# dan11003/tbv_slam_public

Hardware: AMD Instinct MI355X
Metric: radar scan registrations/sec (400x3360 polar) (higher is better)
Workload: dtype u8 filter / f32 search / f64 solve

## Files before the change

include/cfear_hip.h:

```cpp
#ifndef CFEAR_HIP_H
#define CFEAR_HIP_H
#include <stddef.h>
#include <stdint.h>

#ifdef __cplusplus
extern "C" {
#endif

#define CFEAR_ABI_VERSION 1

#define CFEAR_OK 0
#define CFEAR_ERR_INVALID_ARGUMENT (-1)
#define CFEAR_ERR_HIP (-2)
#define CFEAR_ERR_CAPACITY (-3)
#define CFEAR_ERR_TOO_FEW_RESIDUALS (-4)
#define CFEAR_ERR_SOLVER (-5)
#define CFEAR_ERR_EMPTY_CLOUD (-6)
#define CFEAR_ERR_NO_DEVICE (-7)
#define CFEAR_ERR_IO (-8)
#define CFEAR_ERR_FORMAT (-9)

enum cfear_cost_metric { CFEAR_P2P = 0, CFEAR_P2L = 1, CFEAR_P2D = 2 };
enum cfear_loss_type { CFEAR_LOSS_NONE = 0, CFEAR_LOSS_HUBER = 1, CFEAR_LOSS_CAUCHY = 2,
                       CFEAR_LOSS_SOFTLONE = 3, CFEAR_LOSS_COMBINED = 4,
// ... 204 lines not shown
#define CFEAR_SURF_REASON_ROTATION 2u
#define CFEAR_SURF_REASON_POINTS 3u
#define CFEAR_SURF_REASON_CELLS 4u
#define CFEAR_SURF_REASON_ORDER 5u
#define CFEAR_SURF_REASON_ROWS3 6u
#define CFEAR_SURF_PATH_SLAB_COUNT_SHIFT 16
#define CFEAR_SURF_PATH_SLAB_COUNT_MASK 0xFF0000u
int cfear_scan_destroy(cfear_scan* scan);

typedef struct cfear_scan_batch cfear_scan_batch;
int cfear_scan_create_batch(cfear_ctx* ctx, const float* xyzi, const int64_t* offsets, const int32_t* lengths, int32_t n_scans,
                            const cfear_feature_params* par, const double* mots, int32_t max_cells, cfear_scan_batch** out,
                            int32_t* status);
int cfear_scan_batch_size(const cfear_scan_batch* batch);
int cfear_scan_batch_get(const cfear_scan_batch* batch, int32_t i, const cfear_scan** scan);
int cfear_scan_batch_destroy(cfear_scan_batch* batch);

typedef struct cfear_reg_params {
  int32_t cost;
  int32_t loss;
  double loss_limit;
  int32_t weight_opt;
  int32_t max_itr_association;
  int32_t max_itr_solver;
  int32_t min_itr;
  double radius;
  double cov_scale;
  double regularization;
  double score_tolerance;
  int32_t itr;
// ... 717 lines not shown
```

tbv_slam_public_amd/_lib.py:

```python
import ctypes as C
import os

import numpy as np

_HERE = os.path.dirname(os.path.abspath(__file__))
SO_PATH = os.path.join(_HERE, "libcfear_hip.so")

OK = 0
ERR_INVALID_ARGUMENT, ERR_HIP, ERR_CAPACITY = -1, -2, -3
ERR_TOO_FEW_RESIDUALS, ERR_SOLVER, ERR_EMPTY_CLOUD, ERR_NO_DEVICE = -4, -5, -6, -7
ERR_IO, ERR_FORMAT = -8, -9

P2P, P2L, P2D = 0, 1, 2
LOSS = {"None": 0, "Huber": 1, "Cauchy": 2, "SoftLOne": 3, "Combined": 4, "Tukey": 5}
COST = {"P2P": 0, "P2L": 1, "P2D": 2}

SURF_PATH_KIND_MASK, SURF_PATH_FAST, SURF_PATH_SINGLE, SURF_PATH_GLOBAL = 3, 1, 2, 3
SURF_PATH_ROWS, SURF_PATH_K64, SURF_PATH_WFLOAT, SURF_PATH_SLABS, SURF_PATH_READ2 = 0x4, 0x8, 0x10, 0x20, 0x40
SURF_PATH_TIER16, SURF_PATH_TIER4, SURF_PATH_TIER1, SURF_PATH_TOP_BUCKET, SURF_PATH_CEN_SCRATCH = 0x80, 0x100, 0x200, 0x400, 0x800
SURF_PATH_PREPARED, SURF_PATH_REASON_SHIFT, SURF_PATH_REASON_MASK = 0x1000, 13, 0xE000
SURF_REASON_REACH, SURF_REASON_ROTATION, SURF_REASON_POINTS, SURF_REASON_CELLS, SURF_REASON_ORDER, SURF_REASON_ROWS3 = 1, 2, 3, 4, 5, 6
SURF_PATH_SLAB_COUNT_SHIFT, SURF_PATH_SLAB_COUNT_MASK = 16, 0xFF0000


# ... 296 lines not shown
    "cfear_rccl_unique_id", "cfear_rccl_comm_init", "cfear_rccl_comm_destroy",
    "cfear_candidate_pipe_create", "cfear_candidate_pipe_submit", "cfear_candidate_pipe_collect", "cfear_candidate_pipe_destroy", "cfear_candidate_pipe_stats",
    "cfear_eval_params_default", "cfear_eval_trajectories", "cfear_eval_check", "cfear_kitti_read", "cfear_kitti_write",
    "cfear_kitti_from_xyt", "cfear_cen2018_params_default", "cfear_filter_cen2018",
    "cfear_cen2019_params_default", "cfear_filter_cen2019",
    "cfear_logreg_params_default", "cfear_logreg_fit_batch", "cfear_p2p_quality", "cfear_p2p_quality_batch",
    "cfear_cart_params_default", "cfear_polar_to_cartesian", "cfear_cart_quality_batch",
    "cfear_cacfar_plan", "cfear_filter_cacfar_rowkeys", "cfear_kstrong_plan",
    "cfear_closure_params_default", "cfear_closure_candidates_batch",
    "cfear_loop_stats_params_default", "cfear_loop_stats_batch", "cfear_loop_curves_params_default", "cfear_loop_curves_batch",
    "cfear_sync_trajectories", "cfear_tum_write", "cfear_cov_write",
    "cfear_graph_align_batch", "cfear_graph_map_batch", "cfear_graph_string_write", "cfear_graph_output_write",
    "cfear_association_ties_batch", "cfear_scan_closest_ties",
    "cfear_voxel_audit_params_default", "cfear_voxel_order_audit_batch",
    "cfear_cen2019_order_audit",
    "cfear_scan_create_batch", "cfear_scan_batch_size", "cfear_scan_batch_get", "cfear_scan_batch_destroy",
    "cfear_odometry_replay_clouds", "cfear_odometry_replay",
    "cfear_sc_detect_batch",
    "cfear_kstrong_rowkeys_derive",
    "cfear_odometry_grid_plan", "cfear_odometry_grid_create", "cfear_odometry_grid_process", "cfear_odometry_grid_destroy",
]


class RowkeysClass(C.Structure):
    _fields_ = [("image", C.c_int32), ("k_strongest", C.c_int32), ("z_min", C.c_float), ("range_res", C.c_float),
                ("min_distance", C.c_float)]


GRID_STREAM_DTYPE = np.dtype([(n, "<i4") for n in ("sequence", "config", "sweep", "filter_class", "surface_group", "matcher_group",
                                                   "surface_slot", "matcher_slot")])

# ... 254 lines not shown
    L.cfear_sc_detect_sequence.argtypes = [vp, C.POINTER(ScManagerParams), C.POINTER(ScNode), C.c_int32, C.c_int32, C.c_int32,
                                           vp, vp]
    L.cfear_sc_detect_batch.argtypes = [vp, C.POINTER(ScManagerParams), C.POINTER(ScBatch), vp, vp]
    L.cfear_sc_manager_size.argtypes = [vp]
    L.cfear_sc_manager_destroy.argtypes = [vp]
    L.cfear_scan_closest_idx.argtypes = [vp, vp, C.c_int32, C.c_double, vp]
    L.cfear_scan_closest_ties.argtypes = [vp, vp, C.c_int32, C.c_double, vp, vp, vp]
    L.cfear_association_ties_batch.argtypes = [vp, C.POINTER(RegJob), C.c_int32, C.POINTER(RegParams), C.c_int32, vp, vp, C.c_int64]
    L.cfear_voxel_audit_params_default.argtypes = [C.POINTER(VoxelAuditParams)]
    L.cfear_voxel_audit_params_default.restype = None
    L.cfear_voxel_order_audit_batch.argtypes = [vp, vp, vp, vp, C.c_int32, C.POINTER(VoxelAuditParams), vp, vp, C.c_int64, C.POINTER(C.c_int64)]
    L.cfear_scan_surface_path.argtypes = [vp, C.POINTER(C.c_uint32)]
    L.cfear_scan_create_batch.argtypes = [vp, vp, vp, vp, C.c_int32, C.POINTER(FeatureParams), vp, C.c_int32, C.POINTER(vp), vp]
    L.cfear_scan_batch_size.argtypes = [vp]
    L.cfear_scan_batch_get.argtypes = [vp, C.c_int32, C.POINTER(vp)]
    L.cfear_scan_batch_destroy.argtypes = [vp]
    L.cfear_odometry_replay_clouds.argtypes = [vp, C.POINTER(ScCloud), C.POINTER(OdometryParams), vp, vp, C.c_int32, C.c_int32, vp]
    L.cfear_odometry_replay.argtypes = [vp, C.POINTER(PolarDesc), vp, C.POINTER(OdometryParams), vp, vp, C.c_int32, C.c_int32, vp]
    L.cfear_polar_rotate_ccw.argtypes = [vp, vp, C.POINTER(PolarDesc), vp, C.c_int32, C.c_int64]
    L.cfear_verify_params_default.argtypes = [C.POINTER(VerifyParams)]
    L.cfear_verify_params_default.restype = None
    L.cfear_verify_loop_candidates.argtypes = [vp, C.POINTER(VerifyJob), C.c_int32, C.POINTER(VerifyParams), vp]
    L.cfear_verify_apply_constraints.argtypes = [vp, C.c_int32, C.POINTER(VerifyParams), vp]
    L.cfear_verify_by_odometry.argtypes = [vp, C.c_int32, C.c_double, C.c_int32, C.POINTER(C.c_double)]
    L.cfear_get_cost.argtypes = [vp, C.POINTER(vp), C.c_int32, C.POINTER(C.c_double), C.POINTER(RegParams),
                                 C.POINTER(C.c_double), C.POINTER(C.c_double), C.c_int32,
                                 C.POINTER(C.c_int32), C.POINTER(C.c_double)]
    L.cfear_cost_prepare.argtypes = [vp, C.POINTER(vp), C.c_int32, C.POINTER(C.c_double),
                                     C.POINTER(RegParams), C.c_int32, C.POINTER(vp)]
    L.cfear_cost_num_blocks.argtypes = [vp]
# ... 94 lines not shown
```

tbv_slam_public_amd/api.py:

```python
import ctypes as C
import math
import os

import numpy as np

from . import _lib as L


def _is_torch(x):
    return type(x).__module__.startswith("torch")


def _ptr(x):
    if x is None:
        return None, None
    if _is_torch(x):
        assert x.is_contiguous()
        return x.data_ptr(), x
    assert x.flags["C_CONTIGUOUS"]
    return x.ctypes.data, x


def _torch_ready(ctx, *arrays):
    if not any(_is_torch(a) for a in arrays):
# ... 527 lines not shown
            ctx.check(ctx._lib.cfear_scan_batch_get(h, i, C.byref(s)))
            m = None
            if s.value:
                m = MapPointNormal._from_handle(s, ctx)
                m._batch = self
            self._scans.append(m)

    def __len__(self):
        return len(self._scans)

    def __getitem__(self, i):
        return self._scans[i]

    def __iter__(self):
        return iter(self._scans)

    def close(self):
        if getattr(self, "_h", None):
            for m in self._scans:
                if m is not None:
                    m._h, m._batch = None, None
            if getattr(self.ctx, "h", None):
                self.ctx._lib.cfear_scan_batch_destroy(self._h)
            self._h = None

    def __del__(self):
        try:
            self.close()
        except Exception:
            pass
# ... 3149 lines not shown
```

tbv_slam_public_amd/csrc/common.hpp:

```cpp
#pragma once
#include <hip/hip_runtime.h>

#include <cstddef>
#include <cstdint>
#include <cstdio>
#include <cstring>
#include <initializer_list>
#include <map>
#include <string>
#include <type_traits>
#include <vector>

#include "../../include/cfear_hip.h"
#include "batch_tables.hpp"
#include "owned.hpp"
#include "reg_layout.hpp"

#define CFEAR_WAVE 64

template <class T> using DevBuf = Owned<T, hipFree>;
template <class T> using PinnedBuf = Owned<T[], hipHostFree>;
using Event = Owned<std::remove_pointer_t<hipEvent_t>, hipEventDestroy>;
using Stream = Owned<std::remove_pointer_t<hipStream_t>, hipStreamDestroy>;
using GraphExec = Owned<std::remove_pointer_t<hipGraphExec_t>, hipGraphExecDestroy>;
// ... 237 lines not shown
  DevBuf<void> slab;
  ScanView view;
  int32_t n_cells_host;
  uint32_t surf_path = 0;
  int32_t refs = 1;
  cfear_scan_batch* batch = nullptr;
};
void cfear_scan_retain(cfear_scan* scan);
int cfear_scan_release(cfear_scan* scan);

struct cfear_scan_batch {
  cfear_ctx* ctx = nullptr;
  DevBuf<void> arena;
  size_t arena_bytes = 0;
  std::vector<cfear_scan*> scans;
  int32_t live = 0;
  bool released = false;
};
void cfear_scan_batch_free(cfear_scan_batch* b);
int cfear_scan_batch_build(cfear_ctx* ctx, const float* const* clouds, const char* on_host, bool one_buffer, const int32_t* lengths, int n_scans,
                           const cfear_feature_params* par, const double* mots, int max_cells, cfear_scan_batch** out, int32_t* status);

size_t cfear_scan_slab_bytes(int cap);
ScanView cfear_scan_view(void* slab, int cap);
int cfear_scan_alloc(cfear_ctx* ctx, int cap, cfear_scan** out);
int cfear_scan_clone_view(cfear_ctx* ctx, const ScanView& src, int n_cells, cfear_scan** out);

struct cfear_kstrong_fused {
  uint32_t* row_keys = nullptr;
  int32_t* row_valid = nullptr;
// ... 166 lines not shown
```

tbv_slam_public_amd/csrc/surface.hip:

```cpp
#include <cfloat>
#include <cmath>
#include <memory>
#include <type_traits>

#include "common.hpp"
#include "fastmath.hpp"
#include "gridsort.hpp"

namespace {

constexpr int kSurfThreads = kGridSortThreads;
constexpr int kMaxPoints = kGridSortMaxPoints;
constexpr int kMaxGridRows = 4096;
constexpr int kPerThread = kMaxPoints / kSurfThreads;
constexpr size_t kLdsRowbegOff = (size_t)kMaxPoints * 8 + 16;
constexpr size_t kLdsSmallOff = (kLdsRowbegOff + (size_t)(kMaxGridRows + 1) * 4 + 15) / 16 * 16;
constexpr size_t kLdsTotal = kLdsSmallOff + 256 + 64 + 32;

struct SurfJob {
  float4* xyzi;
  const int32_t* n_ptr;
  int32_t n_host;
  int32_t compensate;
  double mot[3];
// ... 218 lines not shown
  if (!cov_reasonable) return 0;
  double n0 = vmin[0], n1 = vmin[1];
  if (n0 * (ox - u0) + n1 * (oy - u1) < 0) { n0 = -n0; n1 = -n1; }
  tc.mean[0] = u0; tc.mean[1] = u1;
  tc.normal[0] = n0; tc.normal[1] = n1;
  tc.cov[0] = c00; tc.cov[1] = c01; tc.cov[2] = c10; tc.cov[3] = c11;
  tc.scale = log(1.0 + condition_number / 2);
  tc.avg_intensity = sum_intensity / (double)m.cnt;
  tc.lmin = lmin; tc.lmax = lmax;
  tc.nsamples = m.cnt;
  tc.valid = 1;
  return 1;
}

constexpr size_t kScanGridLds = (size_t)kScanGridCells * 4 + 128;
__device__ void grid_cells_block(const ScanView& v, int n, uint8_t* lds) {
  const int tid = threadIdx.x, nth = blockDim.x;
  unsigned* cnt = (unsigned*)lds;
  unsigned* ext = cnt + kScanGridCells;
  auto ordered = [](float f) { unsigned u = __float_as_uint(f); return (u >> 31) ? ~u : (u | 0x80000000u); };
  auto unordered = [](unsigned u) { return __uint_as_float((u >> 31) ? (u & 0x7fffffffu) : ~u); };
  if (n > 65535) {
    if (tid == 0) *v.grid_geo = make_float4(0.f, 0.f, 0.f, 0.f);
    return;
  }
  const int np = scan_grid_pad(n);
  unsigned short* cstart = v.grid;
  float2* rec_xy = (float2*)(v.grid + kScanGridStartPad);
  unsigned short* rec_idx = (unsigned short*)(rec_xy + np);
  for (int c = tid; c < kScanGridCells; c += nth) cnt[c] = 0;
  if (tid < 4) ext[tid] = (tid & 1) ? 0u : 0xFFFFFFFFu;
  __syncthreads();
  {
    unsigned xl = 0xFFFFFFFFu, xh = 0u, yl = 0xFFFFFFFFu, yh = 0u;
    for (int i = tid; i < n; i += nth) {
      const g_f32x2 m = gload<g_f32x2>(v.mean_f + i);
      const unsigned ux = ordered(m.x), uy = ordered(m.y);
      xl = min(xl, ux); xh = max(xh, ux); yl = min(yl, uy); yh = max(yh, uy);
    }
    for (int o = 32; o > 0; o >>= 1) {
      xl = min(xl, (unsigned)__shfl_xor((int)xl, o)); xh = max(xh, (unsigned)__shfl_xor((int)xh, o));
      yl = min(yl, (unsigned)__shfl_xor((int)yl, o)); yh = max(yh, (unsigned)__shfl_xor((int)yh, o));
    }
    if ((tid & 63) == 0) { atomicMin(&ext[0], xl); atomicMax(&ext[1], xh); atomicMin(&ext[2], yl); atomicMax(&ext[3], yh); }
  }
  __syncthreads();
  float x0 = 0.f, y0 = 0.f, span = 0.f;
  if (n > 0) {
    x0 = unordered(ext[0]); y0 = unordered(ext[2]);
    span = fmaxf(unordered(ext[1]) - x0, unordered(ext[3]) - y0);
  }
  const float inv = 1.0f / fmaxf(span / (float)kScanGrid * 1.0001f, kScanGridMinEdge);
  auto cell_of = [&](float x, float y) {
    const int cx = min(kScanGrid - 1, max(0, (int)floorf((x - x0) * inv)));
    const int cy = min(kScanGrid - 1, max(0, (int)floorf((y - y0) * inv)));
    return cy * kScanGrid + cx;
  };
  for (int i = tid; i < n; i += nth) { const g_f32x2 m = gload<g_f32x2>(v.mean_f + i); atomicAdd(&cnt[cell_of(m.x, m.y)], 1u); }
  __syncthreads();
  {
    const int per = (kScanGridCells + nth - 1) / nth, c0 = tid * per, c1 = min(kScanGridCells, c0 + per);
    int tot = 0;
    for (int c = c0; c < c1; c++) tot += (int)cnt[c];
    const int incl = wave_incl_scan_i32(tot);
    if ((tid & 63) == 63) ext[4 + (tid >> 6)] = (unsigned)incl;
    __syncthreads();
    int run = incl - tot;
    for (int wv = 0; wv < (tid >> 6); wv++) run += (int)ext[4 + wv];
    for (int c = c0; c < c1; c++) {
      const int k = (int)cnt[c];
      gstore<unsigned short>(cstart + c, (unsigned short)run);
      cnt[c] = (unsigned)run;
      run += k;
    }
    if (tid < kScanGridStartPad - kScanGridCells) gstore<unsigned short>(cstart + kScanGridCells + tid, (unsigned short)n);
  }
  __syncthreads();
  for (int i = tid; i < n; i += nth) {
    const g_f32x2 m = gload<g_f32x2>(v.mean_f + i);
    const unsigned pos = atomicAdd(&cnt[cell_of(m.x, m.y)], 1u);
    gstore<g_f32x2>(rec_xy + pos, m);
    gstore<unsigned short>(rec_idx + pos, (unsigned short)i);
  }
  if (tid < np - n) {
    gstore<g_f32x2>(rec_xy + n + tid, g_f32x2{0.f, 0.f});
    gstore<unsigned short>(rec_idx + n + tid, (unsigned short)0);
  }
  if (tid == 0) gstore<g_f32x4>(v.grid_geo, g_f32x4{x0, y0, inv, 1.f});
}

__global__ __launch_bounds__(kSurfThreads) void scan_grid_kernel(ScanView v) {
  __shared__ __attribute__((aligned(16))) uint8_t smem[kScanGridLds];
  grid_cells_block(v, *v.n_cells, smem);
}

__device__ void surface_big_tail(const SurfJob& job, const SurfCommon& cm, const int job_id, const int n, const int dbx,
                                 const int dby, const int min_bx, const int min_by, uint8_t* smem) {
  int* red_i = (int*)(smem + kLdsSmallOff + 256);
  const int tid = threadIdx.x, wave = tid >> 6, lane = tid & 63;
  const SurfScratch scr = scratch_of(cm.scratch + (size_t)job_id * cm.scratch_stride, cm.scratch_cap);
  const float4* pts = job.xyzi;
  unsigned long long* keys = scr.bigkeys;
  int npad = 1024;
  while (npad < n) npad <<= 1;
  for (int i = tid; i < npad; i += kSurfThreads) {
    unsigned long long key = ~0ull;
    if (i < n) {
      const float4 p = pts[i];
// ... 348 lines not shown
        job.out.mean[off] = make_double2(t.mean[0], t.mean[1]);
        job.out.normal[off] = make_double2(t.normal[0], t.normal[1]);
        job.out.cov[off] = make_double4(t.cov[0], t.cov[1], t.cov[2], t.cov[3]);
        job.out.scale[off] = t.scale;
        job.out.avg_intensity[off] = t.avg_intensity;
        job.out.lambda[off] = make_double2(t.lmin, t.lmax);
        job.out.nsamples[off] = t.nsamples;
      }
    }
    __syncthreads();
    if (tid == 0) { int tot = 0; for (int wv = 0; wv < 16; wv++) tot += red_i[wv]; sh_misc[0] += tot; }
    __syncthreads();
  }
  __threadfence_block();
  __syncthreads();
  grid_cells_block(job.out, min(sh_misc[0], job.out.cap), smem);
  if (tid == 0) {
    const int total = sh_misc[0];
    *job.out.n_cells = total <= job.out.cap ? total : job.out.cap;
    *status = total <= job.out.cap ? CFEAR_OK : CFEAR_ERR_CAPACITY;
    if (cm.ncells_out) cm.ncells_out[job_id] = total <= job.out.cap ? total : job.out.cap;
    if (cm.path_out) cm.path_out[job_id] = path;
  }
}

__global__ __launch_bounds__(kSurfThreads) void surface_points_kernel(const SurfJob* __restrict__ jobs, const SurfCommon cm) {
  extern __shared__ __attribute__((aligned(16))) uint8_t smem[];
  if (!cm.fallback) { surface_points_job(jobs, cm, blockIdx.x, smem); return; }
  const int count = min(cm.fallback[0], cm.n_jobs);
  for (int w = blockIdx.x; w < count; w += gridDim.x) {
    surface_points_job(jobs, cm, cm.fallback[1 + w], smem);
// ... 574 lines not shown
    scr.hdr->n = n; scr.hdr->V = V; scr.hdr->dbx = dbx; scr.hdr->dby = dby;
    scr.hdr->path = path | (n_slabs > 1 ? CFEAR_SURF_PATH_SLABS : 0u) | ((uint32_t)min(n_slabs, 255) << CFEAR_SURF_PATH_SLAB_COUNT_SHIFT);
  }
}

__global__ __launch_bounds__(kFastThreads, 4) void surface_sort_kernel(const SurfJob* __restrict__ jobs, const SurfCommon cm) {
  surface_sort_job<32>(jobs, cm);
}
__global__ __launch_bounds__(kFastThreads, 4) void surface_sort_mixed_kernel(const SurfJob* __restrict__ jobs, const SurfCommon cm) {
  const SurfScratch scr = scratch_of(cm.scratch + (size_t)blockIdx.x * cm.scratch_stride, cm.scratch_cap);
  if (scr.hdr->n > 32 * kFastThreads) surface_sort_job<64>(jobs, cm);
  else surface_sort_job<32>(jobs, cm);
}

constexpr int kFinishThreads = 256;

__global__ __launch_bounds__(kFinishThreads, 5) void surface_finish_kernel(const SurfJob* __restrict__ jobs, const SurfCommon cm) {
  extern __shared__ __attribute__((aligned(16))) uint8_t smem[];
  __shared__ int red_i2[2][kFinishThreads / 64];
  const int tid = threadIdx.x, wave = tid >> 6, lane = tid & 63;
  const int job_id = blockIdx.x;
  const SurfScratch scr = scratch_of(cm.scratch + (size_t)job_id * cm.scratch_stride, cm.scratch_cap);
  if (job_id == 0 && tid == 0) cm.fallback[0] = 0;
  if (scr.hdr->route != kRouteFast) return;
  const SurfJob job = jobs[job_id];
  const int V = scr.hdr->V;
  int run = 0;
  int cnt_next = tid < V ? gload<int32_t>(scr.coff + tid) : 0;
  for (int v0 = 0, rnd = 0; v0 < V; v0 += kFinishThreads, rnd ^= 1) {
    const int v = v0 + tid;
    const int cnt = cnt_next;
    cnt_next = v + kFinishThreads < V ? gload<int32_t>(scr.coff + v + kFinishThreads) : 0;
    TmpCell t;
    int f = 0;
    if (v < V && cnt >= 6) {
      const char* src = (const char*)&scr.tmp[v];
      const g_f64x2 a = gload<g_f64x2>(src), b = gload<g_f64x2>(src + 16), c = gload<g_f64x2>(src + 32);
      const g_f32x2 d = gload<g_f32x2>(src + 48);
      const Moments mo{cnt, a.x, a.y, b.x, b.y, c.x, c.y};
      f = finish_cell(mo, (double)d.x, (double)d.y, cm.origin[0], cm.origin[1], t);
    }
    const int inc = wave_incl_scan_i32(f);
    if (lane == 63) red_i2[rnd][wave] = inc;
    __syncthreads();
    int off = run + inc - f;
    for (int wv = 0; wv < kFinishThreads / 64; wv++) { if (wv < wave) off += red_i2[rnd][wv]; run += red_i2[rnd][wv]; }
    if (f && off < job.out.cap) {
      gstore<g_f32x2>(job.out.mean_f + off, g_f32x2{(float)t.mean[0], (float)t.mean[1]});
      gstore<g_f64x2>(job.out.mean + off, g_f64x2{t.mean[0], t.mean[1]});
      gstore<g_f64x2>(job.out.normal + off, g_f64x2{t.normal[0], t.normal[1]});
      gstore<g_f64x4>(job.out.cov + off, g_f64x4{t.cov[0], t.cov[1], t.cov[2], t.cov[3]});
      gstore<double>(job.out.scale + off, t.scale);
      gstore<double>(job.out.avg_intensity + off, t.avg_intensity);
      gstore<g_f64x2>(job.out.lambda + off, g_f64x2{t.lmin, t.lmax});
      gstore<int32_t>(job.out.nsamples + off, t.nsamples);
    }
  }
  __threadfence_block();
  __syncthreads();
  const int total = run;
  const int cap = min(job.out.cap, cm.finish_keys);
  grid_cells_block(job.out, min(total, cap), smem);
  if (tid == 0) {
    *job.out.n_cells = total <= cap ? total : cap;
    cm.status[job_id] = total <= cap ? CFEAR_OK : CFEAR_ERR_CAPACITY;
    if (cm.ncells_out) cm.ncells_out[job_id] = total <= cap ? total : cap;
    if (cm.path_out) cm.path_out[job_id] = scr.hdr->path;
  }
}

__global__ void cells_to_slab_kernel(const cfear_cell* cells, int n, ScanView v) {
  const int i = blockIdx.x * blockDim.x + threadIdx.x;
  if (i == 0) *v.n_cells = n;
  if (i >= n) return;
  const cfear_cell c = cells[i];
  v.mean_f[i] = make_float2((float)c.mean[0], (float)c.mean[1]);
  v.mean[i] = make_double2(c.mean[0], c.mean[1]);
  v.normal[i] = make_double2(c.normal[0], c.normal[1]);
  v.cov[i] = make_double4(c.cov[0], c.cov[1], c.cov[2], c.cov[3]);
  v.scale[i] = c.scale;
  v.avg_intensity[i] = c.avg_intensity;
  v.lambda[i] = make_double2(c.lambda_min, c.lambda_max);
  v.nsamples[i] = c.nsamples;
}
// ... 71 lines not shown
  cm.range_res = polar ? polar->range_res : 0.0;
  cm.range_off = polar ? polar->range_off : 0.0;
  cm.n_jobs = n_jobs;
  cm.fast_ok = cm.reach == 1 ? 1 : 0;
  const size_t ws_bytes_before = ctx->ws[kWsSurfaceList].bytes;
  cm.fallback = (int32_t*)cfear_workspace(ctx, kWsSurfaceList, ((size_t)n_jobs + 16) * 4);
  if (!cm.fallback) return cfear_set_error(ctx, CFEAR_ERR_HIP, "workspace allocation failed");
  if (ctx->ws[kWsSurfaceList].bytes != ws_bytes_before || ctx->surf_list_dirty)
    CFEAR_HIP_CHECK(ctx, hipMemsetAsync(cm.fallback, 0, 4, ctx->stream));
  ctx->surf_list_dirty = true;
  { const int rc_lds = cfear_allow_lds(ctx, (const void*)surface_points_kernel, cfear_surface_lds_bytes()); if (rc_lds != CFEAR_OK) return rc_lds; }
  { const int rc_lds = cfear_allow_lds(ctx, (const void*)surface_sort_kernel, kFastLds); if (rc_lds != CFEAR_OK) return rc_lds; }
  const bool big_scans = cap_points > kMaxPoints;
  if (big_scans) { const int rc_lds = cfear_allow_lds(ctx, (const void*)surface_sort_mixed_kernel, kFastLds); if (rc_lds != CFEAR_OK) return rc_lds; }
  cm.finish_keys = std::min(max_cell_cap, kMaxPoints);
  const size_t finish_lds = kScanGridLds;
  cm.finish_lds = (uint32_t)finish_lds;
  {
    size_t prep_lds = 0;
    if (polar) {
      const size_t np = (size_t)std::min<long long>((long long)polar->rows * polar->k, kFastMaxPoints);
      prep_lds = (((size_t)(polar->rows + 1) * 4 + 15) & ~(size_t)15) + ((np * 2 + 15) & ~(size_t)15) + (size_t)polar->rows * 16;
      if (prep_lds > 150 * 1024) return cfear_set_error(ctx, CFEAR_ERR_CAPACITY, "%d azimuths exceed the row tables", polar->rows);
      if (prep_lds > 64 * 1024)
        { const int rc_lds = cfear_allow_lds(ctx, (const void*)surface_prep_kernel<true>, prep_lds); if (rc_lds != CFEAR_OK) return rc_lds; }
    }
    ProfScope ps(ctx, "surface_prep");
    if (polar) hipLaunchKernelGGL(surface_prep_kernel<true>, dim3(n_jobs), dim3(kFastThreads), prep_lds, ctx->stream, (const SurfJob*)d_jobs, cm);
    else hipLaunchKernelGGL(surface_prep_kernel<false>, dim3(n_jobs), dim3(kFastThreads), 0, ctx->stream, (const SurfJob*)d_jobs, cm);
  }
  {
// ... 17 lines not shown
    static int calls = 0;
    if (++calls % 40 == 0) {
      (void)hipStreamSynchronize(ctx->stream);
      {
        int32_t nfb = -1;
        (void)hipMemcpy(&nfb, cm.fallback, 4, hipMemcpyDeviceToHost);
        int routes[4] = {0, 0, 0, 0}, prepared = 0;
        for (int j = 0; j < n_jobs; j++) {
          SurfHdr h;
          (void)hipMemcpy(&h, d_scratch + (size_t)j * cm.scratch_stride, sizeof(h), hipMemcpyDeviceToHost);
          if (h.route >= 0 && h.route < 4) routes[h.route]++;
          if (h.route == kRouteFallback) prepared += h.pad[0];
        }
        fprintf(stderr, "surface routes of %d jobs: fast %d  fallback %d (prepared %d)  done %d  prepped %d\n", n_jobs, routes[0], routes[1], prepared, routes[2], routes[3]);
      }
      double acc[9] = {0}, sub[5] = {0}, cel[6] = {0};
      const int m = std::min(n_jobs, 256);
      for (int j = 0; j < m; j++) {
        long long t[24];
        (void)hipMemcpy(t, d_scratch + (size_t)(j * (n_jobs / m)) * cm.scratch_stride + 64, sizeof(t), hipMemcpyDeviceToHost);
        for (int q = 1; q < 9; q++) acc[q] += (double)(t[q] - t[q - 1]);
        sub[0] += (double)(t[9] - t[2]); sub[1] += (double)(t[10] - t[3]);
        sub[2] += (double)(t[16] - t[9]); sub[3] += (double)(t[17] - t[16]); sub[4] += (double)(t[3] - t[17]);
        cel[0] += (double)(t[11] - t[7]); cel[1] += (double)(t[12] - t[11]); cel[2] += (double)(t[13] - t[12]);
        cel[3] += (double)(t[14] - t[13]); cel[4] += (double)(t[15] - t[14]); cel[5] += (double)(t[8] - t[15]);
      }
      fprintf(stderr, "  cells split (last slab, tid 0): stage %.0f  classify+list %.0f  centroids %.0f  16-lane %.0f  4-lane %.0f  1-lane %.0f\n",
              cel[0] / m, cel[1] / m, cel[2] / m, cel[3] / m, cel[4] / m, cel[5] / m);
      fprintf(stderr, "  of hist: clear the bitmap %.0f, first 8 points per thread %.0f, the rest %.0f, barrier %.0f; of scan: word scan + voxel keys %.0f\n",
              sub[0] / m, sub[2] / m, sub[3] / m, sub[4] / m, sub[1] / m);
      fprintf(stderr, "surface_sort phases (cycles, mean of %d jobs): count %.0f  comp+bbox %.0f  hist %.0f  scan %.0f  scatter %.0f  order %.0f  spt %.0f  cells %.0f\n",
              m, acc[1] / m, acc[2] / m, acc[3] / m, acc[4] / m, acc[5] / m, acc[6] / m, acc[7] / m, acc[8] / m);
    }
  }
#endif
  return CFEAR_OK;
}

int cfear_compensate_batch_device(cfear_ctx* ctx, float* d_xyzi, size_t cloud_stride_points, const int32_t* d_n, const double* d_mot,
                                  int n_clouds, int max_points, int ccw) {
  if (n_clouds <= 0) return CFEAR_OK;
// ... 119 lines not shown

int cfear_scan_batch_build(cfear_ctx* ctx, const float* const* clouds, const char* on_host, bool one_buffer, const int32_t* lengths, int n_scans,
                           const cfear_feature_params* par, const double* mots, int max_cells, cfear_scan_batch** out, int32_t* status) {
  *out = nullptr;
  if (max_cells < 1 || max_cells > kMaxPoints)
    return cfear_set_error(ctx, CFEAR_ERR_INVALID_ARGUMENT, "max_cells must be in [1, %d]", kMaxPoints);
  std::vector<int> idx;
  for (int i = 0; i < n_scans; i++) {
    status[i] = lengths[i] == 0 ? CFEAR_ERR_EMPTY_CLOUD : lengths[i] > kScanCreateMaxPoints ? CFEAR_ERR_CAPACITY : CFEAR_OK;
    if (status[i] == CFEAR_OK) idx.push_back(i);
  }
  CFEAR_HIP_CHECK(ctx, hipSetDevice(ctx->device));
  std::unique_ptr<cfear_scan_batch, int (*)(cfear_scan_batch*)> b(new cfear_scan_batch(), cfear_scan_batch_destroy);
  b->ctx = ctx;
  b->scans.assign((size_t)n_scans, nullptr);
  const size_t slab_bytes = cfear_scan_slab_bytes(max_cells);
  b->arena_bytes = slab_bytes * (size_t)n_scans;
  if (ctx->free_arena.bytes >= b->arena_bytes) {
    b->arena = std::move(ctx->free_arena.p);
    b->arena_bytes = ctx->free_arena.bytes;
    ctx->free_arena.bytes = 0;
  } else if (!(b->arena = dev_alloc<void>(b->arena_bytes))) {
    return cfear_set_error(ctx, CFEAR_ERR_HIP, "scan batch: hipMalloc of %zu bytes failed", b->arena_bytes);
  }
  std::vector<int32_t> hst;
  for (size_t c0 = 0; c0 < idx.size();) {
    size_t c1 = c0;
    int cap_points = 0;
    while (c1 < idx.size()) {
      const int cp = std::max(cap_points, lengths[idx[c1]]);
// ... 42 lines not shown
  std::vector<const float*> clouds((size_t)n_scans);
  for (int i = 0; i < n_scans; i++) clouds[(size_t)i] = xyzi ? xyzi + 4 * offsets[i] : nullptr;
  const std::vector<char> on_host((size_t)n_scans, (char)(any && !cfear_is_device_ptr(xyzi)));
  return cfear_scan_batch_build(ctx, clouds.data(), on_host.data(), true, lengths, n_scans, par, mots, max_cells, out, status);
}

extern "C" int cfear_scan_batch_size(const cfear_scan_batch* batch) { return batch ? (int)batch->scans.size() : CFEAR_ERR_INVALID_ARGUMENT; }

extern "C" int cfear_scan_batch_get(const cfear_scan_batch* batch, int32_t i, const cfear_scan** scan) {
  if (!batch || !scan) return CFEAR_ERR_INVALID_ARGUMENT;
  *scan = nullptr;
  if (i < 0 || (size_t)i >= batch->scans.size())
    return cfear_set_error(batch->ctx, CFEAR_ERR_INVALID_ARGUMENT, "scan %d of a batch of %zu", i, batch->scans.size());
  *scan = batch->scans[(size_t)i];
  return CFEAR_OK;
}

extern "C" int cfear_scan_batch_destroy(cfear_scan_batch* batch) {
  if (!batch) return CFEAR_OK;
  batch->released = true;
  for (cfear_scan*& s : batch->scans) {
    cfear_scan* h = s;
    s = nullptr;
    if (h && --h->refs == 0) { delete h; batch->live--; }
  }
  if (batch->live == 0) cfear_scan_batch_free(batch);
  return CFEAR_OK;
}

extern "C" int cfear_scan_surface_path(const cfear_scan* scan, uint32_t* path) {
// ... 102 lines not shown
```

Before: 1.429 million.

## Compact surviving voxels before finishing cells and reuse means in grid build

The surface_finish kernel now runs a pre-pass that ballots over voxel counts in chunks, compacting the indices of voxels with at least six samples into an LDS list. The finishing rounds then iterate only over that dense list, prefetching the next moments while computing the current ones. The kernel also keeps the first finished float means in LDS and accumulates the grid bounding box during finishing, so the grid build skips its extent pass and global re-reads for those cells. This raises LDS use per workgroup (guarded by a static_assert for five groups per CU), and the change also adds a batch peek_cells API and optional timing stamps.

```diff
diff --git a/include/cfear_hip.h b/include/cfear_hip.h
--- a/include/cfear_hip.h
+++ b/include/cfear_hip.h
@@ -242,6 +242,7 @@
                             int32_t* status);
 int cfear_scan_batch_size(const cfear_scan_batch* batch);
 int cfear_scan_batch_get(const cfear_scan_batch* batch, int32_t i, const cfear_scan** scan);
+int cfear_scan_batch_peek_cells(const cfear_scan_batch* batch, int32_t i, cfear_cell* out_host, int32_t cap);
 int cfear_scan_batch_destroy(cfear_scan_batch* batch);
 
 typedef struct cfear_reg_params {
diff --git a/tbv_slam_public_amd/_lib.py b/tbv_slam_public_amd/_lib.py
--- a/tbv_slam_public_amd/_lib.py
+++ b/tbv_slam_public_amd/_lib.py
@@ -334,7 +334,7 @@
     "cfear_association_ties_batch", "cfear_scan_closest_ties",
     "cfear_voxel_audit_params_default", "cfear_voxel_order_audit_batch",
     "cfear_cen2019_order_audit",
-    "cfear_scan_create_batch", "cfear_scan_batch_size", "cfear_scan_batch_get", "cfear_scan_batch_destroy",
+    "cfear_scan_create_batch", "cfear_scan_batch_size", "cfear_scan_batch_get", "cfear_scan_batch_peek_cells", "cfear_scan_batch_destroy",
     "cfear_odometry_replay_clouds", "cfear_odometry_replay",
     "cfear_sc_detect_batch",
     "cfear_kstrong_rowkeys_derive",
@@ -619,6 +619,7 @@
     L.cfear_scan_create_batch.argtypes = [vp, vp, vp, vp, C.c_int32, C.POINTER(FeatureParams), vp, C.c_int32, C.POINTER(vp), vp]
     L.cfear_scan_batch_size.argtypes = [vp]
     L.cfear_scan_batch_get.argtypes = [vp, C.c_int32, C.POINTER(vp)]
+    L.cfear_scan_batch_peek_cells.argtypes = [vp, C.c_int32, vp, C.c_int32]
     L.cfear_scan_batch_destroy.argtypes = [vp]
     L.cfear_odometry_replay_clouds.argtypes = [vp, C.POINTER(ScCloud), C.POINTER(OdometryParams), vp, vp, C.c_int32, C.c_int32, vp]
     L.cfear_odometry_replay.argtypes = [vp, C.POINTER(PolarDesc), vp, C.POINTER(OdometryParams), vp, vp, C.c_int32, C.c_int32, vp]
diff --git a/tbv_slam_public_amd/api.py b/tbv_slam_public_amd/api.py
--- a/tbv_slam_public_amd/api.py
+++ b/tbv_slam_public_amd/api.py
@@ -565,6 +565,13 @@
 
     def __iter__(self):
         return iter(self._scans)
+
+    def peek_cells(self, i, cap=16384):
+        out = np.zeros(max(int(cap), 1), L.CELL_DTYPE)
+        n = self.ctx._lib.cfear_scan_batch_peek_cells(self._h, int(i), out.ctypes.data, out.shape[0])
+        if n < 0:
+            self.ctx.check(n)
+        return out[:n]
 
     def close(self):
         if getattr(self, "_h", None):
diff --git a/tbv_slam_public_amd/csrc/common.hpp b/tbv_slam_public_amd/csrc/common.hpp
--- a/tbv_slam_public_amd/csrc/common.hpp
+++ b/tbv_slam_public_amd/csrc/common.hpp
@@ -275,6 +275,8 @@
   DevBuf<void> arena;
   size_t arena_bytes = 0;
   std::vector<cfear_scan*> scans;
+  std::vector<char> served;
+  int32_t max_cells = 0;
   int32_t live = 0;
   bool released = false;
 };
diff --git a/tbv_slam_public_amd/csrc/surface.hip b/tbv_slam_public_amd/csrc/surface.hip
--- a/tbv_slam_public_amd/csrc/surface.hip
+++ b/tbv_slam_public_amd/csrc/surface.hip
@@ -256,12 +256,20 @@
 }
 
 constexpr size_t kScanGridLds = (size_t)kScanGridCells * 4 + 128;
-__device__ void grid_cells_block(const ScanView& v, int n, uint8_t* lds) {
+__device__ __forceinline__ unsigned grid_ordered(float f) { const unsigned u = __float_as_uint(f); return (u >> 31) ? ~u : (u | 0x80000000u); }
+__device__ __forceinline__ float grid_unordered(unsigned u) { return __uint_as_float((u >> 31) ? (u & 0x7fffffffu) : ~u); }
+constexpr int kGridKeep = 4;
+template <bool KEPT>
+__device__ void grid_cells_block(const ScanView& v, int n, uint8_t* lds, const float2* lmean = nullptr, int n_lmean = 0,
+                                 const unsigned* pre_ext = nullptr) {
   const int tid = threadIdx.x, nth = blockDim.x;
   unsigned* cnt = (unsigned*)lds;
   unsigned* ext = cnt + kScanGridCells;
-  auto ordered = [](float f) { unsigned u = __float_as_uint(f); return (u >> 31) ? ~u : (u | 0x80000000u); };
-  auto unordered = [](unsigned u) { return __uint_as_float((u >> 31) ? (u & 0x7fffffffu) : ~u); };
+  constexpr int keep = KEPT ? kGridKeep : 0;
+  auto mean_at = [&](int i) {
+    if (KEPT && i < n_lmean) { const float2 m = lmean[i]; return g_f32x2{m.x, m.y}; }
+    return gload<g_f32x2>(v.mean_f + i);
+  };
   if (n > 65535) {
     if (tid == 0) *v.grid_geo = make_float4(0.f, 0.f, 0.f, 0.f);
     return;
@@ -275,9 +283,10 @@
   __syncthreads();
   {
     unsigned xl = 0xFFFFFFFFu, xh = 0u, yl = 0xFFFFFFFFu, yh = 0u;
-    for (int i = tid; i < n; i += nth) {
+    if (KEPT) { xl = pre_ext[0]; xh = pre_ext[1]; yl = pre_ext[2]; yh = pre_ext[3]; }
+    for (int i = tid; !KEPT && i < n; i += nth) {
       const g_f32x2 m = gload<g_f32x2>(v.mean_f + i);
-      const unsigned ux = ordered(m.x), uy = ordered(m.y);
+      const unsigned ux = grid_ordered(m.x), uy = grid_ordered(m.y);
       xl = min(xl, ux); xh = max(xh, ux); yl = min(yl, uy); yh = max(yh, uy);
     }
     for (int o = 32; o > 0; o >>= 1) {
@@ -289,8 +298,8 @@
   __syncthreads();
   float x0 = 0.f, y0 = 0.f, span = 0.f;
   if (n > 0) {
-    x0 = unordered(ext[0]); y0 = unordered(ext[2]);
-    span = fmaxf(unordered(ext[1]) - x0, unordered(ext[3]) - y0);
+    x0 = grid_unordered(ext[0]); y0 = grid_unordered(ext[2]);
+    span = fmaxf(grid_unordered(ext[1]) - x0, grid_unordered(ext[3]) - y0);
   }
   const float inv = 1.0f / fmaxf(span / (float)kScanGrid * 1.0001f, kScanGridMinEdge);
   auto cell_of = [&](float x, float y) {
@@ -298,7 +307,13 @@
     const int cy = min(kScanGrid - 1, max(0, (int)floorf((y - y0) * inv)));
     return cy * kScanGrid + cx;
   };
-  for (int i = tid; i < n; i += nth) { const g_f32x2 m = gload<g_f32x2>(v.mean_f + i); atomicAdd(&cnt[cell_of(m.x, m.y)], 1u); }
+  int kept[keep > 0 ? keep : 1];
+#pragma unroll
+  for (int k = 0; k < keep; k++) {
+    const int i = tid + k * nth;
+    if (i < n) { const g_f32x2 m = mean_at(i); kept[k] = cell_of(m.x, m.y); atomicAdd(&cnt[kept[k]], 1u); }
+  }
+  for (int i = tid + keep * nth; i < n; i += nth) { const g_f32x2 m = mean_at(i); atomicAdd(&cnt[cell_of(m.x, m.y)], 1u); }
   __syncthreads();
   {
     const int per = (kScanGridCells + nth - 1) / nth, c0 = tid * per, c1 = min(kScanGridCells, c0 + per);
@@ -318,8 +333,17 @@
     if (tid < kScanGridStartPad - kScanGridCells) gstore<unsigned short>(cstart + kScanGridCells + tid, (unsigned short)n);
   }
   __syncthreads();
-  for (int i = tid; i < n; i += nth) {
-    const g_f32x2 m = gload<g_f32x2>(v.mean_f + i);
+#pragma unroll
+  for (int k = 0; k < keep; k++) {
+    const int i = tid + k * nth;
+    if (i < n) {
+      const unsigned pos = atomicAdd(&cnt[kept[k]], 1u);
+      gstore<g_f32x2>(rec_xy + pos, mean_at(i));
+      gstore<unsigned short>(rec_idx + pos, (unsigned short)i);
+    }
+  }
+  for (int i = tid + keep * nth; i < n; i += nth) {
+    const g_f32x2 m = mean_at(i);
     const unsigned pos = atomicAdd(&cnt[cell_of(m.x, m.y)], 1u);
     gstore<g_f32x2>(rec_xy + pos, m);
     gstore<unsigned short>(rec_idx + pos, (unsigned short)i);
@@ -333,7 +357,7 @@
 
 __global__ __launch_bounds__(kSurfThreads) void scan_grid_kernel(ScanView v) {
   __shared__ __attribute__((aligned(16))) uint8_t smem[kScanGridLds];
-  grid_cells_block(v, *v.n_cells, smem);
+  grid_cells_block<false>(v, *v.n_cells, smem);
 }
 
 __device__ void surface_big_tail(const SurfJob& job, const SurfCommon& cm, const int job_id, const int n, const int dbx,
@@ -712,7 +736,7 @@
   }
   __threadfence_block();
   __syncthreads();
-  grid_cells_block(job.out, min(sh_misc[0], job.out.cap), smem);
+  grid_cells_block<false>(job.out, min(sh_misc[0], job.out.cap), smem);
   if (tid == 0) {
     const int total = sh_misc[0];
     *job.out.n_cells = total <= job.out.cap ? total : job.out.cap;
@@ -1317,60 +1341,129 @@
 }
 
 constexpr int kFinishThreads = 256;
+constexpr int kFinishWaves = kFinishThreads / 64;
+constexpr int kFinishList = 1024;
+constexpr int kFinishChunkRounds = 8;
+constexpr int kFinishChunk = kFinishChunkRounds * kFinishThreads;
+constexpr int kFinishMeans = kGridKeep * kFinishThreads;
+constexpr size_t kFinishListOff = kScanGridLds;
+constexpr size_t kFinishMeansOff = kFinishListOff + (size_t)kFinishList * sizeof(int2);
+constexpr size_t kFinishLds = kFinishMeansOff + (size_t)kFinishMeans * sizeof(float2);
+static_assert(kFinishListOff % 16 == 0 && 5 * (kFinishLds + 256) <= 160 * 1024, "five surface_finish workgroups per CU");
+static_assert(kFinishWaves == 4, "the pre-pass keeps a round's four wave totals in one int4");
 
 __global__ __launch_bounds__(kFinishThreads, 5) void surface_finish_kernel(const SurfJob* __restrict__ jobs, const SurfCommon cm) {
   extern __shared__ __attribute__((aligned(16))) uint8_t smem[];
-  __shared__ int red_i2[2][kFinishThreads / 64];
+  __shared__ int red_i2[2][kFinishWaves];
+  __shared__ int4 wave_tot[kFinishChunkRounds];
+  int2* list = (int2*)(smem + kFinishListOff);
+  float2* lmean = (float2*)(smem + kFinishMeansOff);
   const int tid = threadIdx.x, wave = tid >> 6, lane = tid & 63;
   const int job_id = blockIdx.x;
   const SurfScratch scr = scratch_of(cm.scratch + (size_t)job_id * cm.scratch_stride, cm.scratch_cap);
   if (job_id == 0 && tid == 0) cm.fallback[0] = 0;
   if (scr.hdr->route != kRouteFast) return;
   const SurfJob job = jobs[job_id];
-  const int V = scr.hdr->V;
+  const int V = __builtin_amdgcn_readfirstlane(scr.hdr->V);
+  const int cap = min(job.out.cap, cm.finish_keys);
+#ifdef CFEAR_SURF_TIMING
+#define FINISH_STAMPS ((long long*)((char*)scr.hdr + 64))
+  if (tid == 0) FINISH_STAMPS[18] = FINISH_STAMPS[19] = FINISH_STAMPS[20] = 0;
+  unsigned t_mark = (unsigned)__builtin_readcyclecounter();
+#define FINISH_LAP(i) do { const unsigned t_now = (unsigned)__builtin_readcyclecounter(); if (tid == 0) FINISH_STAMPS[i] += (long long)(t_now - t_mark); t_mark = t_now; } while (0)
+#else
+#define FINISH_LAP(i) do { } while (0)
+#endif
   int run = 0;
-  int cnt_next = tid < V ? gload<int32_t>(scr.coff + tid) : 0;
-  for (int v0 = 0, rnd = 0; v0 < V; v0 += kFinishThreads, rnd ^= 1) {
-    const int v = v0 + tid;
-    const int cnt = cnt_next;
-    cnt_next = v + kFinishThreads < V ? gload<int32_t>(scr.coff + v + kFinishThreads) : 0;
-    TmpCell t;
-    int f = 0;
-    if (v < V && cnt >= 6) {
-      const char* src = (const char*)&scr.tmp[v];
-      const g_f64x2 a = gload<g_f64x2>(src), b = gload<g_f64x2>(src + 16), c = gload<g_f64x2>(src + 32);
-      const g_f32x2 d = gload<g_f32x2>(src + 48);
-      const Moments mo{cnt, a.x, a.y, b.x, b.y, c.x, c.y};
-      f = finish_cell(mo, (double)d.x, (double)d.y, cm.origin[0], cm.origin[1], t);
-    }
-    const int inc = wave_incl_scan_i32(f);
-    if (lane == 63) red_i2[rnd][wave] = inc;
+  unsigned xl = 0xFFFFFFFFu, xh = 0u, yl = 0xFFFFFFFFu, yh = 0u;
+  auto request = [&](int e, int m, int& cnt, g_f64x2& a, g_f64x2& b, g_f64x2& c, g_f32x2& d) {
+    if (e < m) {
+      const int2 ent = list[e];
+      const char* src = (const char*)&scr.tmp[ent.x];
+      cnt = ent.y;
+      a = gload<g_f64x2>(src); b = gload<g_f64x2>(src + 16); c = gload<g_f64x2>(src + 32); d = gload<g_f32x2>(src + 48);
+    }
+  };
+  for (int c0 = 0, base = 0; c0 < V;) {
+    if (c0 + base > 0) __syncthreads();
+    int cnts[kFinishChunkRounds];
+#pragma unroll
+    for (int r = 0; r < kFinishChunkRounds; r++) {
+      const int v = c0 + r * kFinishThreads + tid;
+      cnts[r] = v < V ? gload<int32_t>(scr.coff + v) : 0;
+    }
+    unsigned long long cand[kFinishChunkRounds];
+#pragma unroll
+    for (int r = 0; r < kFinishChunkRounds; r++) {
+      cand[r] = __ballot(cnts[r] >= 6);
+      if (lane == 0) ((int*)&wave_tot[r])[wave] = __popcll(cand[r]);
+    }
     __syncthreads();
-    int off = run + inc - f;
-    for (int wv = 0; wv < kFinishThreads / 64; wv++) { if (wv < wave) off += red_i2[rnd][wv]; run += red_i2[rnd][wv]; }
-    if (f && off < job.out.cap) {
-      gstore<g_f32x2>(job.out.mean_f + off, g_f32x2{(float)t.mean[0], (float)t.mean[1]});
-      gstore<g_f64x2>(job.out.mean + off, g_f64x2{t.mean[0], t.mean[1]});
-      gstore<g_f64x2>(job.out.normal + off, g_f64x2{t.normal[0], t.normal[1]});
-      gstore<g_f64x4>(job.out.cov + off, g_f64x4{t.cov[0], t.cov[1], t.cov[2], t.cov[3]});
-      gstore<double>(job.out.scale + off, t.scale);
-      gstore<double>(job.out.avg_intensity + off, t.avg_intensity);
-      gstore<g_f64x2>(job.out.lambda + off, g_f64x2{t.lmin, t.lmax});
-      gstore<int32_t>(job.out.nsamples + off, t.nsamples);
-    }
-  }
-  __threadfence_block();
-  __syncthreads();
+    int pos = -base;
+#pragma unroll
+    for (int r = 0; r < kFinishChunkRounds; r++) {
+      const int4 t = wave_tot[r];
+      const int p = pos + (wave > 0 ? t.x : 0) + (wave > 1 ? t.y : 0) + (wave > 2 ? t.z : 0) +
+                    (int)__builtin_amdgcn_mbcnt_hi((unsigned)(cand[r] >> 32), __builtin_amdgcn_mbcnt_lo((unsigned)cand[r], 0u));
+      if (cnts[r] >= 6 && (unsigned)p < (unsigned)kFinishList) list[p] = make_int2(c0 + r * kFinishThreads + tid, cnts[r]);
+      pos += t.x + t.y + t.z + t.w;
+    }
+    const int left = pos;
+    const int m = min(left, kFinishList);
+    __syncthreads();
+    FINISH_LAP(18);
+    int cnt = 0;
+    g_f64x2 a = {0.0, 0.0}, b = {0.0, 0.0}, c = {0.0, 0.0};
+    g_f32x2 d = {0.f, 0.f};
+    request(tid, m, cnt, a, b, c, d);
+    for (int k0 = 0, rnd = 0; k0 < m; k0 += kFinishThreads, rnd ^= 1) {
+      TmpCell t;
+      int f = 0;
+      if (k0 + tid < m) {
+        const Moments mo{cnt, a.x, a.y, b.x, b.y, c.x, c.y};
+        f = finish_cell(mo, (double)d.x, (double)d.y, cm.origin[0], cm.origin[1], t);
+      }
+      request(k0 + kFinishThreads + tid, m, cnt, a, b, c, d);
+      const int inc = wave_incl_scan_i32(f);
+      if (lane == 63) red_i2[rnd][wave] = inc;
+      __syncthreads();
+      int off = run + inc - f;
+      for (int wv = 0; wv < kFinishWaves; wv++) { if (wv < wave) off += red_i2[rnd][wv]; run += red_i2[rnd][wv]; }
+      if (f && off < job.out.cap) {
+        const float mfx = (float)t.mean[0], mfy = (float)t.mean[1];
+        gstore<g_f32x2>(job.out.mean_f + off, g_f32x2{mfx, mfy});
+        gstore<g_f64x2>(job.out.mean + off, g_f64x2{t.mean[0], t.mean[1]});
+        gstore<g_f64x2>(job.out.normal + off, g_f64x2{t.normal[0], t.normal[1]});
+        gstore<g_f64x4>(job.out.cov + off, g_f64x4{t.cov[0], t.cov[1], t.cov[2], t.cov[3]});
+        gstore<double>(job.out.scale + off, t.scale);
+        gstore<double>(job.out.avg_intensity + off, t.avg_intensity);
+        gstore<g_f64x2>(job.out.lambda + off, g_f64x2{t.lmin, t.lmax});
+        gstore<int32_t>(job.out.nsamples + off, t.nsamples);
+        if (off < kFinishMeans) lmean[off] = make_float2(mfx, mfy);
+        if (off < cap) {
+          const unsigned ux = grid_ordered(mfx), uy = grid_ordered(mfy);
+          xl = min(xl, ux); xh = max(xh, ux); yl = min(yl, uy); yh = max(yh, uy);
+        }
+      }
+    }
+    FINISH_LAP(19);
+    if (left > kFinishList) base += kFinishList;
+    else { base = 0; c0 += kFinishChunk; }
+  }
   const int total = run;
-  const int cap = min(job.out.cap, cm.finish_keys);
-  grid_cells_block(job.out, min(total, cap), smem);
+  const int n_grid = min(total, cap);
+  if (n_grid > kFinishMeans) __threadfence_block();
+  const unsigned pre_ext[4] = {xl, xh, yl, yh};
+  grid_cells_block<true>(job.out, n_grid, smem, lmean, kFinishMeans, pre_ext);
   if (tid == 0) {
     *job.out.n_cells = total <= cap ? total : cap;
     cm.status[job_id] = total <= cap ? CFEAR_OK : CFEAR_ERR_CAPACITY;
     if (cm.ncells_out) cm.ncells_out[job_id] = total <= cap ? total : cap;
     if (cm.path_out) cm.path_out[job_id] = scr.hdr->path;
-  }
-}
+    FINISH_LAP(20);
+  }
+}
+#undef FINISH_LAP
 
 __global__ void cells_to_slab_kernel(const cfear_cell* cells, int n, ScanView v) {
   const int i = blockIdx.x * blockDim.x + threadIdx.x;
@@ -1472,7 +1565,7 @@
   const bool big_scans = cap_points > kMaxPoints;
   if (big_scans) { const int rc_lds = cfear_allow_lds(ctx, (const void*)surface_sort_mixed_kernel, kFastLds); if (rc_lds != CFEAR_OK) return rc_lds; }
   cm.finish_keys = std::min(max_cell_cap, kMaxPoints);
-  const size_t finish_lds = kScanGridLds;
+  const size_t finish_lds = kFinishLds;
   cm.finish_lds = (uint32_t)finish_lds;
   {
     size_t prep_lds = 0;
@@ -1520,7 +1613,7 @@
         }
         fprintf(stderr, "surface routes of %d jobs: fast %d  fallback %d (prepared %d)  done %d  prepped %d\n", n_jobs, routes[0], routes[1], prepared, routes[2], routes[3]);
       }
-      double acc[9] = {0}, sub[5] = {0}, cel[6] = {0};
+      double acc[9] = {0}, sub[5] = {0}, cel[6] = {0}, fin[3] = {0};
       const int m = std::min(n_jobs, 256);
       for (int j = 0; j < m; j++) {
         long long t[24];
@@ -1530,7 +1623,9 @@
         sub[2] += (double)(t[16] - t[9]); sub[3] += (double)(t[17] - t[16]); sub[4] += (double)(t[3] - t[17]);
         cel[0] += (double)(t[11] - t[7]); cel[1] += (double)(t[12] - t[11]); cel[2] += (double)(t[13] - t[12]);
         cel[3] += (double)(t[14] - t[13]); cel[4] += (double)(t[15] - t[14]); cel[5] += (double)(t[8] - t[15]);
-      }
+        fin[0] += (double)t[18]; fin[1] += (double)t[19]; fin[2] += (double)t[20];
+      }
+      fprintf(stderr, "surface_finish phases (cycles, tid 0): pre-pass %.0f  dense rounds %.0f  grid + status %.0f\n", fin[0] / m, fin[1] / m, fin[2] / m);
       fprintf(stderr, "  cells split (last slab, tid 0): stage %.0f  classify+list %.0f  centroids %.0f  16-lane %.0f  4-lane %.0f  1-lane %.0f\n",
               cel[0] / m, cel[1] / m, cel[2] / m, cel[3] / m, cel[4] / m, cel[5] / m);
       fprintf(stderr, "  of hist: clear the bitmap %.0f, first 8 points per thread %.0f, the rest %.0f, barrier %.0f; of scan: word scan + voxel keys %.0f\n",
@@ -1680,6 +1775,9 @@
   std::unique_ptr<cfear_scan_batch, int (*)(cfear_scan_batch*)> b(new cfear_scan_batch(), cfear_scan_batch_destroy);
   b->ctx = ctx;
   b->scans.assign((size_t)n_scans, nullptr);
+  b->served.assign((size_t)n_scans, 0);
+  for (int i : idx) b->served[(size_t)i] = 1;
+  b->max_cells = max_cells;
   const size_t slab_bytes = cfear_scan_slab_bytes(max_cells);
   b->arena_bytes = slab_bytes * (size_t)n_scans;
   if (ctx->free_arena.bytes >= b->arena_bytes) {
@@ -1752,6 +1850,17 @@
     return cfear_set_error(batch->ctx, CFEAR_ERR_INVALID_ARGUMENT, "scan %d of a batch of %zu", i, batch->scans.size());
   *scan = batch->scans[(size_t)i];
   return CFEAR_OK;
+}
+
+extern "C" int cfear_scan_batch_peek_cells(const cfear_scan_batch* batch, int32_t i, cfear_cell* out_host, int32_t cap) {
+  if (!batch || !out_host) return CFEAR_ERR_INVALID_ARGUMENT;
+  if (i < 0 || (size_t)i >= batch->scans.size() || !batch->served[(size_t)i])
+    return cfear_set_error(batch->ctx, CFEAR_ERR_INVALID_ARGUMENT, "scan %d of a batch of %zu had no job", i, batch->scans.size());
+  cfear_scan view;
+  view.ctx = batch->ctx;
+  view.view = cfear_scan_view((char*)batch->arena.get() + (size_t)i * cfear_scan_slab_bytes(batch->max_cells), batch->max_cells);
+  view.n_cells_host = -1;
+  return cfear_scan_get_cells(&view, out_host, cap);
 }
 
 extern "C" int cfear_scan_batch_destroy(cfear_scan_batch* batch) {
```

After: 1.440 million (median of 6 runs). No clear change (+0.7%).
